# FrancisTheCat/raytracing_c

Hardware: AMD Instinct MI355X
Metric: Mray/s (higher is better)
Workload: dtype f32; 1 GPU; helmet.glb 1920x1080, 256 spp, 8 bounces (BASELINE.json configs[2]); partition=single GPU

## Files before the change

include/rt_hip.h:

```cpp
#ifndef RT_HIP_H
#define RT_HIP_H

#include "rt_raytracer.h"
#include "rt_materials.h"

#ifdef __cplusplus
extern "C" {
#endif

extern char const *rt_last_error(void);
extern void        rt_clear_error(void);

extern int rt_init(int device);

extern int rt_set_devices(i32 n_devices, i32 rehearse);
extern i32 rt_device_count(void);


extern void rt_set_seed(u32 seed);
extern u32  rt_get_seed(void);


typedef struct RT_Device_Scene RT_Device_Scene;

// ... 121 lines not shown


typedef struct {
  f32 alpha;
  i32 max_history;
  f32 normal_tolerance, plane_tolerance;
  i32 demodulate;
} RT_Temporal_Params;

typedef struct { f32 *color, *length, *coverage, *normal, *position; } RT_History_Planes;

extern i64 rt_temporal_history_bytes(i32 width, i32 height);
extern int rt_temporal_accumulate(i32 width, i32 height, RT_Temporal_Params const *params, Camera const *camera,
                                  Camera const *previous_camera, void const *d_color, void const *d_coverage, void const *d_albedo,
                                  void const *d_normal, void const *d_position, void const *d_history_in, void *d_history_out,
                                  void *d_out, void *d_length, void *d_image, void *stream);
extern int rt_temporal_accumulate_host(i32 width, i32 height, RT_Temporal_Params const *params, Camera const *camera,
                                       Camera const *previous_camera, f32 const *color, RT_Features const *planes,
                                       RT_History_Planes const *history_in, RT_History_Planes const *history_out, f32 *out,
                                       f32 *length, u8 *image);

typedef struct RT_History RT_History;
extern RT_History *rt_history_create(i32 width, i32 height);
extern int         rt_history_reset(RT_History *history);
extern void        rt_history_destroy(RT_History *history);

extern int rt_render_temporal(Scene const *scene, Image const *image, isize samples, isize max_bounces, RT_History *history,
                              RT_Temporal_Params const *temporal_params, RT_Guided_Params const *guided_params, f32 *linear_noisy,
                              f32 *linear_out, f32 *length);

extern int rt_get_counters(RT_Counters *out);
extern int rt_get_skipped_root_visits(u64 *out);
extern int rt_get_leafless_paths(u64 *out);

typedef struct {
  f32 stamp_ms, upload_ms, enqueue_ms, gpu_prep_ms, gpu_path_ms, gpu_resolve_ms, gpu_copy_ms, total_ms;
  f32 verify_ms;
  f32 gather_ms;
  i32 n_devices;
  i32 slowest_device;
} RT_Frame_Timing;
extern int rt_get_frame_timing(RT_Frame_Timing *out);

extern f32 rt_last_kernel_ms(void);

extern void rt_kernel_timing_reset(void);
extern f32  rt_kernel_timing_mean_ms(i32 *n_launches);

extern int rt_math_contract(void);


#ifdef __cplusplus
}
#endif

#endif
```

raytracing_c_amd/csrc/rt_dev.hip.h:

```cpp
#ifndef RT_DEV_HIP_H
#define RT_DEV_HIP_H

#include <hip/hip_runtime.h>
#include <stdint.h>

#include "rt_device.h"
#include "../../include/rt_math.h"

#define RT_BLOCK_WAVES 4
#define RT_BLOCK_THREADS (RT_BLOCK_WAVES * 64)

#define CNT_PATHS 0
#define CNT_RAYS 1
#define CNT_NODES 2
#define CNT_LEAVES 3
#define CNT_SHADES 4
#define CNT_BG 5
#define CNT_TEXTURED 6
#define CNT_SKIPPED_ROOT 7

struct Ray3 {
  rt_v3 o, d;
  float inv_x, inv_y, inv_z;
  bool  fast;
};

__device__ __forceinline__ rt_v3 slab_bias3(const Ray3 &r) {
#ifdef RT_MATH_NO_FMA
  return rt_v3_make(0.0f, 0.0f, 0.0f);
#else
  float px, py, pz;
  asm volatile("v_mul_f32 %0, %1, %2" : "=v"(px) : "v"(r.o.x), "v"(r.inv_x));
  asm volatile("v_mul_f32 %0, %1, %2" : "=v"(py) : "v"(r.o.y), "v"(r.inv_y));
  asm volatile("v_mul_f32 %0, %1, %2" : "=v"(pz) : "v"(r.o.z), "v"(r.inv_z));
  return rt_v3_make(-px, -py, -pz);
#endif
}

struct HitRec {
  float t;
  int   tri;
  float u, v;
};

struct LaneCounters {
  uint32_t rays, nodes, leaves, shades, bgs, textured, paths;
};

enum {
  LG_S_ITER = 0, LG_ENV_X, LG_ENV_L, LG_SHADE_X, LG_SHADE_L, LG_PSTORE_X, LG_PSTORE_L, LG_PLOAD_X, LG_PLOAD_L, LG_ACCUM_X, LG_ACCUM_L,
  LG_REGEN_X, LG_REGEN_L, LG_START_X, LG_START_L, LG_PRIM_X, LG_PRIM_L, LG_TILE_X, LG_JOIN_X, LG_FLUSH_X, LG_GRAB_X, LG_ROUND_X, LG_TRAV_CALLS,
  LG_NFULL_X, LG_NFULL_L, LG_NFULL_CAM, LG_NGLOB_X, LG_NGLOB_L, LG_NEXACT_X, LG_NEXACT_L, LG_CULLMASK_X, LG_PYRCHK_X, LG_NODE_WAIT_L,
  LG_NFEW0_X, LG_NFEW1_X, LG_NFEW2_X, LG_NFEW3_X, LG_NFEW4_X, LG_NFEW0_L, LG_NFEW1_L, LG_NFEW2_L, LG_NFEW3_L, LG_NFEW4_L,
  LG_LEAF_X, LG_LEAF_L, LG_LEAF_CAM, LG_POP_X, LG_POP_L, LG_POP_UP_L, LG_POP_RETEST_L, LG_POP_CAM, LG_POP_UP_X, LG_POP_RETEST_X, LG_POP_DONE_L,
  LG_CYC_S, LG_CYC_NODE, LG_CYC_LEAF, LG_CYC_POP, LG_CYC_WAVE, LG_CYC_TILE,
  LG_SKY_X, LG_SKY_L, LG_CYC_SKY,
  LG_CYC_COPY, LG_CYC_JOIN, LG_CYC_DRAIN, LG_DRAIN_X, LG_DRAIN_L, LG_CYC_FLUSH,
  LG_N
};
#define RT_LEDGER_ROW 128
#ifdef RT_LEDGER
__device__ __forceinline__ int lane_now();
__device__ __forceinline__ void lg_add(uint32_t *lg, int slot, uint32_t n) {
  if (lane_now() == 0 && n != 0u) __hip_atomic_fetch_add(lg + slot, n, __ATOMIC_RELAXED, __HIP_MEMORY_SCOPE_AGENT);
}
#define LG(slot, n) lg_add(lg, (slot), (uint32_t)(n))
#define LG_ARG , lg
#else
#define LG(slot, n) ((void)0)
#define LG_ARG
#endif
#ifdef RT_LEDGER_MARKS
#define LGM(name) asm volatile("; LEDGER_MARK " name)
#else
#define LGM(name) ((void)0)
#endif
#if defined(RT_LEDGER) && RT_LEDGER >= 2
#define LGT0() const unsigned long long lg_t0 = __builtin_amdgcn_s_memtime()
#define LGT1(slot) LG((slot), (uint32_t)((__builtin_amdgcn_s_memtime() - lg_t0) >> 4))
#define LGD0(n_live) do { if (!lg_drain_t0) { lg_drain_t0 = __builtin_amdgcn_s_memtime(); LG(LG_DRAIN_X, 1); LG(LG_DRAIN_L, (n_live)); } } while (0)
#define LGD1() do { if (lg_drain_t0) { LG(LG_CYC_DRAIN, (uint32_t)((__builtin_amdgcn_s_memtime() - lg_drain_t0) >> 4)); lg_drain_t0 = 0ull; } } while (0)
#else
#define LGT0() ((void)0)
#define LGT1(slot) ((void)0)
#define LGD0(n_live) ((void)0)
#define LGD1() ((void)0)
#endif

__device__ __forceinline__ float4 ld4(const float *base, int idx4) {
  return reinterpret_cast<const float4 *>(base)[idx4];
// ... 778 lines not shown

__device__ __forceinline__ uint32_t pyramid_cull_mask(const float4 *lds_nodes, const float *pyr, int node) {
  const int lane = lane_now();
  const float *nb = reinterpret_cast<const float *>(lds_nodes + lds_node_f4(node)) + (lane & 7);
  const float *pl = pyr + ((lane >> 3) & 3) * 4;
  const float ox = pyr[16], oy = pyr[17], oz = pyr[18];
  const float mnx = nb[0], mny = nb[8], mnz = nb[16], mxx = nb[24], mxy = nb[32], mxz = nb[40];
  const float nx = pl[0], ny = pl[1], nz = pl[2];
  const bool empty = mnx == 0.0f && mny == 0.0f && mnz == 0.0f && mxx == 0.0f && mxy == 0.0f && mxz == 0.0f;
  const float lox = nx * (mnx - ox), hix = nx * (mxx - ox), loy = ny * (mny - oy), hiy = ny * (mxy - oy);
  const float loz = nz * (mnz - oz), hiz = nz * (mxz - oz);
  const float nearest = fminf(lox, hix) + fminf(loy, hiy) + fminf(loz, hiz);
  const float extent = fmaxf(fabsf(lox), fabsf(hix)) + fmaxf(fabsf(loy), fabsf(hiy)) + fmaxf(fabsf(loz), fabsf(hiz));
  const float coarse = fabsf(nx) * (fabsf(ox) + fmaxf(fabsf(mnx), fabsf(mxx))) + fabsf(ny) * (fabsf(oy) + fmaxf(fabsf(mny), fabsf(mxy))) +
                       fabsf(nz) * (fabsf(oz) + fmaxf(fabsf(mnz), fabsf(mxz)));
  const bool outside = empty || nearest > 1e-3f * extent + 1e-6f * coarse;
  const uint32_t m = (uint32_t)__ballot(outside);
  return (m | (m >> 8) | (m >> 16) | (m >> 24)) & 0xFFu;
}

__device__ __forceinline__ float slab_entry_ordered(const Ray3 &r, const rt_v3 &bs, const char *nbase, int k, int nx, int ny, int nz, float t_max) {
  const char *b = nbase + k * 4;
  const float sx = rt_slab_t_fast(*reinterpret_cast<const float *>(b + nx), r.o.x, r.inv_x, bs.x);
  const float bx = rt_slab_t_fast(*reinterpret_cast<const float *>(b + (96 - nx)), r.o.x, r.inv_x, bs.x);
  const float sy = rt_slab_t_fast(*reinterpret_cast<const float *>(b + 32 + ny), r.o.y, r.inv_y, bs.y);
  const float by = rt_slab_t_fast(*reinterpret_cast<const float *>(b + 32 + (96 - ny)), r.o.y, r.inv_y, bs.y);
  const float sz = rt_slab_t_fast(*reinterpret_cast<const float *>(b + 64 + nz), r.o.z, r.inv_z, bs.z);
  const float bz = rt_slab_t_fast(*reinterpret_cast<const float *>(b + 64 + (96 - nz)), r.o.z, r.inv_z, bs.z);
  const float t_minv = fmax_hw(RT_EPS, fmax_hw(sx, fmax_hw(sy, sz)));
  const float t_maxv = fmin_hw(t_max, fmin_hw(bx, fmin_hw(by, bz)));
  return (t_minv < t_maxv) ? t_minv : RT_INF;
}

__device__ __forceinline__ uint32_t node_enter_few(const Ray3 &r, const float4 *lds_nodes, int node, uint32_t surv,
                                                   float hit_t) {
  const char *nbase = reinterpret_cast<const char *>(lds_nodes + lds_node_f4(node));
  const int nx = (as_i(r.inv_x) >> 31) & 96, ny = (as_i(r.inv_y) >> 31) & 96, nz = (as_i(r.inv_z) >> 31) & 96;
  const rt_v3 bs = slab_bias3(r);
  const int n = (int)__popc(surv);
  const int k0 = (int)__builtin_ctz(surv);
  const int e0 = as_i(slab_entry_ordered(r, bs, nbase, k0, nx, ny, nz, hit_t));
  const uint32_t f0 = 1u - (((uint32_t)e0 + 0x00800000u) >> 31);
  LGM("nfew_ret1");
  if (n == 1) return (uint32_t)k0 | (f0 << 24);
  surv &= surv - 1u;
  const int k1 = (int)__builtin_ctz(surv);
  const int e1 = as_i(slab_entry_ordered(r, bs, nbase, k1, nx, ny, nz, hit_t));
  const uint32_t f1 = 1u - (((uint32_t)e1 + 0x00800000u) >> 31);
  LGM("nfew_two");
  if (n == 2) {
    const bool swap = e1 < e0;
    const uint32_t first = swap ? (uint32_t)k1 : (uint32_t)k0, second = swap ? (uint32_t)k0 : (uint32_t)k1;
    return first | (second << 3) | ((f0 + f1) << 24);
  }
  LGM("nfew_ret2");
  surv &= surv - 1u;
  const int k2 = (int)__builtin_ctz(surv);
  const int e2 = as_i(slab_entry_ordered(r, bs, nbase, k2, nx, ny, nz, hit_t));
  const uint32_t f2 = 1u - (((uint32_t)e2 + 0x00800000u) >> 31);
  int e3 = 0x7F800000, k3 = 0;
  uint32_t f3 = 0;
  LGM("nfew_four_begin");
  if (n == 4) {
    surv &= surv - 1u;
    k3 = (int)__builtin_ctz(surv);
      e3 = as_i(slab_entry_ordered(r, bs, nbase, k3, nx, ny, nz, hit_t));
    f3 = 1u - (((uint32_t)e3 + 0x00800000u) >> 31);
  }
  LGM("nfew_four_end");
  const int e[4] = {e0, e1, e2, e3};
  const int kk[4] = {k0, k1, k2, k3};
  int rank[4] = {0, 1, 2, 3};
#pragma unroll
  for (int j = 0; j < 4; j++) {
#pragma unroll
    for (int k = j + 1; k < 4; k++) {
      int kb = (int)((uint32_t)(e[k] - e[j]) >> 31);
      rank[j] += kb;
      rank[k] -= kb;
    }
  }
  uint32_t w = 0;
#pragma unroll
  for (int j = 0; j < 4; j++) w |= (uint32_t)kk[j] << (3 * rank[j]);
  return w | ((f0 + f1 + f2 + f3) << 24);
}

__device__ __forceinline__ uint32_t pyramid_cull_tris(const float *leaves, const float *pyr, int g) {
  const int lane = lane_now();
  const float *tb = leaves + (size_t)g * 72 + (lane & 7);
  const float *pl = pyr + ((lane >> 3) & 3) * 4;
  const float ox = pyr[16], oy = pyr[17], oz = pyr[18];
  const float nx = pl[0], ny = pl[1], nz = pl[2];
  const float ax = tb[0], e1x = tb[8], e2x = tb[16], ay = tb[24], e1y = tb[32], e2y = tb[40], az = tb[48], e1z = tb[56], e2z = tb[64];
  bool outside = true;
#pragma unroll
  for (int v = 0; v < 3; v++) {
    const float vx = v == 0 ? ax : (v == 1 ? ax + e1x : ax + e2x);
    const float vy = v == 0 ? ay : (v == 1 ? ay + e1y : ay + e2y);
    const float vz = v == 0 ? az : (v == 1 ? az + e1z : az + e2z);
    const float px = nx * (vx - ox), py = ny * (vy - oy), pz = nz * (vz - oz);
    const float val = px + py + pz;
    const float extent = fabsf(px) + fabsf(py) + fabsf(pz);
    const float coarse = fabsf(nx) * (fabsf(ox) + fabsf(vx)) + fabsf(ny) * (fabsf(oy) + fabsf(vy)) + fabsf(nz) * (fabsf(oz) + fabsf(vz));
    outside = outside && (val > 1e-3f * extent + 1e-6f * coarse);
  }
  const uint32_t m = (uint32_t)__ballot(outside);
  return (m | (m >> 8) | (m >> 16) | (m >> 24)) & 0xFFu;
}

template <bool SHORT_DIV>
__device__ __forceinline__ void tri_test_uniform(const Ray3 &r, rt_v3 a, rt_v3 edge1, rt_v3 edge2, int k, float &best, float &bu, float &bv, int &bi) {
  rt_v3 rxe2 = rt_v3_cross(r.d, edge2);
  float det = rt_v3_dot(edge1, rxe2);
  float inv_det = SHORT_DIV ? rcp_leaf(det) : 1.0f / det;
  rt_v3 s = rt_v3_sub(r.o, a);
  rt_v3 sxe1 = rt_v3_cross(s, edge1);
  float u = inv_det * rt_v3_dot(s, rxe2);
  float v = inv_det * rt_v3_dot(r.d, sxe1);
// ... 21 lines not shown
  }
  if (best < hit.t) {
    hit.t = best;
    hit.tri = g * 8 + bi;
    hit.u = bu;
    hit.v = bv;
    return true;
  }
  return false;
}

typedef const RT_KParams __attribute__((address_space(4))) *RT_KArgs;
__device__ __forceinline__ RT_KArgs cold_args() {
  RT_KArgs p = (RT_KArgs)__builtin_amdgcn_kernarg_segment_ptr();
  asm volatile("" : "+s"(p));
  return p;
}

struct TravState {
  int      phase, level, node, child;
  uint32_t cur, dirty, live;
  HitRec   hit;
};

template <bool LDSN, bool SHORT_DIV, bool PYRAMID, bool ANY = false>
__device__ __forceinline__ void traversal_blocks(const RT_KParams &P, float4 *smem, const float4 *lds_nodes, uint32_t *perm,
                                                 const int lane, const int n_lds, const int pyr_nodes, const int pyr_off,
                                                 const int leaf_level, const int exit_lanes, const int n_trav0, const Ray3 &ray,
                                                 const bool is_cam, int &phase, int &level, int &node, int &child, uint32_t &cur,
                                                 uint32_t &dirty, uint32_t &live, HitRec &hit, uint32_t &w_nodes, uint32_t &w_leaves,
                                                 uint32_t *lg = nullptr) {
  static_assert(!(ANY && PYRAMID), "the pyramid-culled leaf block has no any-hit exit");
  LG(LG_TRAV_CALLS, 1);
  for (;;) {
    LGM("round_begin");
    const unsigned long long maskN = __ballot(phase == PH_NODE);
    const int nN = (int)__popcll(maskN);
    const int nL = (int)__popcll(__ballot(phase == PH_LEAF));
    if (nN + nL == 0 || n_trav0 - (nN + nL) >= exit_lanes) break;
    LG(LG_ROUND_X, 1);

    if (nL >= nN) {
      LGT0();
      LGM("leaf_begin");
      LG(LG_LEAF_X, 1); LG(LG_LEAF_L, nL);
#ifdef RT_LEDGER
      LG(LG_LEAF_CAM, __popcll(__ballot(phase == PH_LEAF && is_cam)));
#endif
      w_leaves += (uint32_t)nL;
      bool leaf_done = false;
      if (PYRAMID && pyr_nodes > 0) {
        const unsigned long long maskL = __ballot(phase == PH_LEAF);
        const unsigned long long camL = maskL & __ballot(is_cam);
        if (camL != 0ull) {
          const int c0 = __builtin_amdgcn_readlane(child, (int)__builtin_ctzll(camL));
          const int nG = (int)__popcll(camL & __ballot(child == c0));
          const int g0 = c0 - P.last_row_offset;
          if (nG * RT_PYR_DEN >= nL * RT_PYR_NUM && nG >= RT_PYR_MIN && (uint32_t)g0 < 0x800000u) {
            float *pyr = lds_at(smem, pyr_off);
            uint32_t *slot = reinterpret_cast<uint32_t *>(pyr) + 24 + (g0 & 7);
            const uint32_t key = 0x800000u | (uint32_t)g0;
            const uint32_t ce = (uint32_t)__builtin_amdgcn_readfirstlane((int)*slot);
            uint32_t cull;
            if ((ce >> 8) == key) {
              cull = ce & 0xFFu;
            } else {
              cull = pyramid_cull_tris(P.leaves, pyr, g0);
              if (lane_now() == 0) *slot = (key << 8) | cull;
            }
            if (__popc(0xFFu & ~cull) <= RT_LEAF_CULL_MAX) {
              w_leaves -= (uint32_t)(nL - nG);
              if (phase == PH_LEAF && is_cam && child == c0) {
                if (leaf_test_uniform<SHORT_DIV>(P, ray, g0, 0xFFu & ~cull, hit)) dirty = 0xFFFFFFFFu;
                phase = PH_POP;
              }
              leaf_done = true;
            }
          }
        }
// ... 18 lines not shown
        if (LDSN && all_fast && camN != 0ull) {
          const int c0 = __builtin_amdgcn_readlane(child, (int)__builtin_ctzll(camN));
          const int nG = (int)__popcll(camN & __ballot(child == c0));
          LG(LG_PYRCHK_X, 1);
          if (c0 < pyr_nodes && nG * RT_PYR_DEN >= nN * RT_PYR_NUM && nG >= RT_PYR_MIN) {
            float *pyr = lds_at(smem, pyr_off);
            uint32_t *slot = reinterpret_cast<uint32_t *>(pyr) + 32 + (c0 & 31);
            const uint32_t ce = (uint32_t)__builtin_amdgcn_readfirstlane((int)*slot);
            if ((ce >> 8) == (uint32_t)c0 + 1u) {
              surv = 0xFFu & ~ce;
            } else {
              LG(LG_CULLMASK_X, 1);
              LGM("cullmask_begin");
              const uint32_t cull = pyramid_cull_mask(lds_nodes, pyr, c0);
              if (lane_now() == 0) *slot = (((uint32_t)c0 + 1u) << 8) | cull;
              surv = 0xFFu & ~cull;
              LGM("cullmask_end");
            }
            if (__popc(surv) > 4) surv = 0xFFFFu;
            else {
              in_blk = phase == PH_NODE && is_cam && child == c0; w_nodes -= (uint32_t)(nN - nG);
#ifdef RT_LEDGER
              {
                const int ns = (int)__popc(surv);
                LG(LG_NFEW0_X, ns == 0); LG(LG_NFEW1_X, ns == 1); LG(LG_NFEW2_X, ns == 2); LG(LG_NFEW3_X, ns == 3); LG(LG_NFEW4_X, ns == 4);
                LG(LG_NFEW0_L, ns == 0 ? nG : 0); LG(LG_NFEW1_L, ns == 1 ? nG : 0); LG(LG_NFEW2_L, ns == 2 ? nG : 0);
                LG(LG_NFEW3_L, ns == 3 ? nG : 0); LG(LG_NFEW4_L, ns == 4 ? nG : 0); LG(LG_NODE_WAIT_L, nN - nG);
              }
#endif
            }
          }
        }
      }
      if (in_blk) {
        if (level >= 0) {
          perm[level * 64 + lane] = cur;
          live = (cur >> 24) ? (live | (1u << level)) : (live & ~(1u << level));
        }
        node = child;
        level += 1;
        if (PYRAMID && surv <= 0xFFu) {
          LGM("nfew_begin");
          cur = surv ? node_enter_few(ray, lds_nodes, node, surv, hit.t) : 0u;
          LGM("nfew_end");
        } else if (all_fast) {
          if (LDSN && __ballot(node >= n_lds) == 0) {
            LG(LG_NFULL_X, 1); LG(LG_NFULL_L, nN);
#ifdef RT_LEDGER
            LG(LG_NFULL_CAM, __popcll(maskN & __ballot(is_cam)));
#endif
            LGM("nfull_begin");
            cur = node_enter<true, NODE_LDS_ORDERED>(P, ray, node, hit.t, lds_nodes);
            LGM("nfull_end");
          } else {
            LG(LG_NGLOB_X, 1); LG(LG_NGLOB_L, nN);
            LGM("nglob_begin");
            cur = node_enter<true, NODE_GLOBAL>(P, ray, node, hit.t, lds_nodes);
            LGM("nglob_end");
          }
        } else if (ray.fast) {
          LGM("nexact_begin");
          LG(LG_NEXACT_X, 1); LG(LG_NEXACT_L, nN);
          cur = node_enter<true, NODE_GLOBAL>(P, ray, node, hit.t, lds_nodes);
        } else {
          cur = node_enter<false, NODE_GLOBAL>(P, ray, node, hit.t, lds_nodes);
        }
// ... 115 lines not shown
```

raytracing_c_amd/csrc/rt_device.h:

```cpp
#ifndef RT_DEVICE_H
#define RT_DEVICE_H

#include <stdint.h>

#define RT_NODE_F4   12
#define RT_LEAF_F4   18
#define RT_TRI_F4     7
#define RT_MAT_F4     9
#define RT_MAT_FLOATS 36
#define RT_MAX_DEPTH  8

#define RT_LDS_BYTES            (160 * 1024)
#define RT_LDS_NODE_BYTES       208
#define RT_LDS_TABLE_BYTES      64
#define RT_LDS_PERM_LEVEL_BYTES 256
#define RT_LDS_ACC_TILE_BYTES   1536

#define RT_MAT_DISNEY 0
#define RT_MAT_DEBUG  1

#define RT_TILE      8
#define RT_TILE_PIX  64

#define RT_PARK_RECORD_DWORDS (18 * 128)
#define RT_N_COUNTERS 137
#define RT_CNT_LEAFLESS 136



typedef struct {
  uint32_t offset;
  int32_t  width, height, stride;
} RT_DTexture;
#define RT_TEX_TILE_INDEX(x, y, tpr) ((((y) >> 2) * (tpr) + ((x) >> 2)) * 16 + (((y) & 3) << 2) + ((x) & 3))

typedef struct RT_KView {
  float    cam[3][4];
  float    focal_length;
  uint32_t seed;
  uint32_t pad[2];
} RT_KView;

typedef struct {
  const float    *nodes;
  const float    *leaves;
  const float    *tris;
  const float    *mats;
  const RT_DTexture *textures;
  const uint32_t *texels;
  int32_t depth;
  int32_t last_row_offset;
  int32_t bg_texture;
  int32_t n_nodes;
  float cam[3][4];
  float focal_length;
  float inv_width, inv_height, aspect;
  int32_t width, height, samples, max_bounces;
  int32_t sample_first, sample_end;
  uint32_t seed;
// ... 93 lines not shown
```

raytracing_c_amd/csrc/rt_kernels.hip:

```cpp

#include "rt_dev.hip.h"


#ifdef RT_LEDGER
#define RT_LEDGER_WAVES 8192
__device__ uint32_t g_ledger[RT_LEDGER_WAVES * RT_LEDGER_ROW];
__global__ void rt_ledger_reduce_kernel(unsigned long long *counters) {
  const int slot = threadIdx.x;
  if (slot >= LG_N || slot >= RT_LEDGER_ROW) return;
  unsigned long long sum = 0ull;
  for (int w = 0; w < RT_LEDGER_WAVES; w++) sum += g_ledger[w * RT_LEDGER_ROW + slot];
  counters[8 + slot] = sum;
}
#endif

typedef const RT_KView __attribute__((address_space(4))) *RT_KViewP;
template <bool VIEWS> struct CamSrc { typedef RT_KArgs type; };
template <> struct CamSrc<true> { typedef RT_KViewP type; };

template <int WAVES, bool LDSN, int MIN_WAVES_PER_SIMD, bool SHORT_DIV, bool VIEWS>
__global__ __launch_bounds__(WAVES * 64, MIN_WAVES_PER_SIMD) void rt_path_kernel_stream(RT_KParams P) {
  extern __shared__ float4 smem[];
  const int lane = threadIdx.x & 63;
  const int wave = threadIdx.x >> 6;
  const int n_lds = LDSN ? P.n_lds_nodes : 0;
  const float4 *lds_nodes = smem;
  const int perm_f4 = (P.depth > 0 ? P.depth : 1) * 16;
  float4 *wave_base = smem + n_lds * RT_LDS_NODE_F4 + wave * (perm_f4 + 96);
  uint32_t *perm = reinterpret_cast<uint32_t *>(wave_base);
  unsigned long long *acc = reinterpret_cast<unsigned long long *>(wave_base + perm_f4);
  const int acc_off = (n_lds * RT_LDS_NODE_F4 + __builtin_amdgcn_readfirstlane(wave) * (perm_f4 + 96) + perm_f4) * 16;
  const int pyr_off = (n_lds * RT_LDS_NODE_F4 + __builtin_amdgcn_readfirstlane(wave) * (perm_f4 + 96) + perm_f4 - 16) * 16;

#ifdef RT_LEDGER
  uint32_t *lg = g_ledger + (size_t)__builtin_amdgcn_readfirstlane((int)blockIdx.x * WAVES + wave) * RT_LEDGER_ROW;
  const unsigned long long lg_wave_t0 = __builtin_amdgcn_s_memtime();
#if RT_LEDGER >= 2
  unsigned long long lg_drain_t0 = 0ull;
#endif
#endif
  pow24_lds_init((int)threadIdx.x);
  if (LDSN) {
    LGT0();
    const float4 *g = reinterpret_cast<const float4 *>(P.nodes);
    for (int i = threadIdx.x; i < n_lds * 12; i += WAVES * 64) {
      int nd = i / 12, q = i - nd * 12;
      smem[nd * RT_LDS_NODE_F4 + q] = g[i];
    }
    __syncthreads();
    LGT1(LG_CYC_COPY);
  } else {
    __syncthreads();
  }

  acc[lane] = 0ull;
  acc[lane + 64] = 0ull;
  acc[lane + 128] = 0ull;

  uint32_t w_paths = 0, w_rays = 0, w_nodes = 0, w_leaves = 0, w_shades = 0, w_bgs = 0, w_tex = 0;
  const unsigned long long t_wave_start = cold_args()->wave_times ? __builtin_amdgcn_s_memrealtime() : 0ull;
  uint32_t n_tiles_done = 0;
  unsigned long long t_last_grab = 0ull;

  const int shift = P.chunk_shift;
  const int unit_paths = 2 << shift;
  const uint32_t n_chunks_tile = (uint32_t)P.n_chunks_tile;
  const int leaf_level = P.depth - 1;
  const int thresh = P.sched_thresh;
  const int drain_thresh = P.drain_thresh;
  const int pyr_nodes = LDSN ? P.pyr_nodes : 0;
  const int wave_id = (int)blockIdx.x * WAVES + wave;

  bool queue_open = true;
  int  steal_tries = 0;

  for (;;) {
    LGT0();
    LGM("tile_begin");
    int tile_idx = -1;
    if (queue_open) {
      RT_KArgs A = cold_args();
      uint32_t pos = 0;
      if (lane == 0) pos = atomicAdd(A->work_head, 1u);
      pos = (uint32_t)__builtin_amdgcn_readfirstlane((int)pos);
      const uint32_t *order = A->order;
      if (pos < (uint32_t)A->n_tiles) tile_idx = order ? (int)order[pos] : (int)pos;
      else queue_open = false;
    }
    if (tile_idx < 0) {
      if (steal_tries >= RT_STEAL_TRIES) break;
// ... 105 lines not shown
      if (lane < 40) reinterpret_cast<uint32_t *>(pyr)[24 + lane] = 0u;
      bool may_hit = false;
      if (lane < 8) {
        const float *nb = P.nodes + lane;
        rt_v3 lo = rt_v3_make(nb[0] - o.x, nb[8] - o.y, nb[16] - o.z);
        rt_v3 hi = rt_v3_make(nb[24] - o.x, nb[32] - o.y, nb[40] - o.z);
        const bool empty = nb[0] == 0.0f && nb[8] == 0.0f && nb[16] == 0.0f && nb[24] == 0.0f && nb[32] == 0.0f && nb[40] == 0.0f;
        bool outside = empty;
#pragma unroll
        for (int q = 0; q < 4; q++) {
          rt_v3 n = pn[q];
          float lox = n.x * lo.x, hix = n.x * hi.x, loy = n.y * lo.y, hiy = n.y * hi.y, loz = n.z * lo.z, hiz = n.z * hi.z;
          float nearest = fminf(lox, hix) + fminf(loy, hiy) + fminf(loz, hiz);
          float extent = fmaxf(fabsf(lox), fabsf(hix)) + fmaxf(fabsf(loy), fabsf(hiy)) + fmaxf(fabsf(loz), fabsf(hiz));
          float coarse = fabsf(n.x) * (fabsf(o.x) + fmaxf(fabsf(nb[0]), fabsf(nb[24]))) + fabsf(n.y) * (fabsf(o.y) + fmaxf(fabsf(nb[8]), fabsf(nb[32]))) +
                         fabsf(n.z) * (fabsf(o.z) + fmaxf(fabsf(nb[16]), fabsf(nb[40])));
          if (nearest > 1e-3f * extent + 1e-6f * coarse) outside = true;
        }
        may_hit = !outside;
      }
      tile_root_miss = __ballot(may_hit) == 0ull;
    }
#define RT_LEAFLESS_MAX 8
    int n_list = 0;
    int ll_levels = leaf_level, ll_nodes = pyr_nodes, ll_leaf0 = P.last_row_offset;
    asm volatile("" : "+s"(ll_levels), "+s"(ll_nodes), "+s"(ll_leaf0));
    if (ll_levels >= 1 && ll_nodes > 0 && !tile_root_miss) {
      const float *pyr = lds_at(smem, pyr_off);
      uint32_t *list = reinterpret_cast<uint32_t *>(lds_at(smem, pyr_off) - ll_levels * (RT_LDS_PERM_LEVEL_BYTES / 4));
      n_list = 1;
      for (int head = 0; head < n_list; head++) {
        const int nd = head ? __builtin_amdgcn_readfirstlane((int)list[RT_LEAFLESS_MAX + head]) : 0;
        const uint32_t surv = 0xFFu & ~pyramid_cull_mask(lds_nodes, pyr, nd);
        if (surv) {
          const int ns = (int)__popc(surv);
          if (8 * nd + 1 >= ll_leaf0 || 8 * nd + 8 >= ll_nodes || ns > 4 || n_list + ns > RT_LEAFLESS_MAX) { n_list = 0; break; }
          const int k = lane_now();
          if (k < 8 && ((surv >> k) & 1u)) {
            const int at = n_list + (int)__popc(surv & ((1u << k) - 1u));
            list[at] = (uint32_t)(nd * RT_LDS_NODE_BYTES + k * 4) | ((uint32_t)head << 20) | 0x80000000u;
            list[RT_LEAFLESS_MAX + at] = (uint32_t)(8 * nd + 1 + k);
          }
          n_list += ns;
        }
      }
    }
    const uint32_t rays_before = w_rays;
    LG(LG_TILE_X, 1);
    LGM("tile_end");
    LGT1(LG_CYC_TILE);

    int   phase = PH_NEED;
    int   pix = 0, bounce = 0;
    uint32_t rng = 0;
    Ray3  ray;
    ray_setup(ray, rt_v3_make(0, 0, 0), rt_v3_make(0, 0, 1));
    rt_v3 tint = rt_v3_make(1, 1, 1), emis = rt_v3_make(0, 0, 0);
    int   level = -1, node = 0, child = 0;
    uint32_t cur = 0, dirty = 0, live = 0;
    HitRec hit;
    hit.t = RT_INF; hit.tri = -1; hit.u = 0; hit.v = 0;

    bool tile_open = true;
    int  c_next = 0, c_end = 0, c_x0 = 0, c_y = 0, c_pix0 = 0, c_s0 = 0;
    uint32_t u_cur = 0, u_end = 0, grab = queue_open ? (uint32_t)cold_args()->grab_max : 1u;
    bool took_any = false;
// ... 294 lines not shown
          { const int n_pr = (int)__popcll(__ballot(got)); LG(LG_PRIM_X, n_pr != 0); LG(LG_PRIM_L, n_pr); LG(LG_REGEN_L, n_pr); }
#endif
          LGM("prim_begin");
          if (got) {
            typename CamSrc<VIEWS>::type S;
            if constexpr (VIEWS) S = vrec; else S = A;
            pix = gp;
            bounce = 0;
            rng = rt_path_seed(S->seed, (uint32_t)(gx + gy * width), (uint32_t)gs);
            PrimaryParams PP;
#pragma unroll
            for (int i = 0; i < 3; i++)
#pragma unroll
              for (int j = 0; j < 4; j++) PP.cam[i][j] = S->cam[i][j];
            PP.focal_length = S->focal_length; PP.inv_width = A->inv_width; PP.inv_height = A->inv_height; PP.aspect = A->aspect;
            primary_ray(PP, gx, gy, gs, org, dir);
            tint = rt_v3_make(1, 1, 1);
            emis = rt_v3_make(0, 0, 0);
            start = true;
            fresh = true;
          }
          LGM("prim_end");
        }
        bool skip_root = false;
#ifdef RT_LEDGER
        { const int n_st = (int)__popcll(__ballot(start)); LG(LG_START_X, n_st != 0); LG(LG_START_L, n_st); }
#endif
        LGM("start_begin");
        if (start) {
          ray_setup<SHORT_DIV>(ray, org, dir);
          hit.t = RT_INF; hit.tri = -1; hit.u = 0; hit.v = 0;
          dirty = 0;
          live = 0;
          cur = 0;
          level = -1;
          node = 0;
          child = (leaf_level >= 0) ? 0 : P.last_row_offset;
          phase = (leaf_level >= 0) ? PH_NODE : PH_LEAF;
          skip_root = fresh && tile_root_miss && ray.fast;
          if (skip_root) phase = PH_MISS;
        }
        LGM("start_end");
        w_rays += (uint32_t)__popcll(__ballot(start));
        {
          const uint32_t n_skip = (uint32_t)__popcll(__ballot(skip_root));
          w_nodes += n_skip;
          if (n_skip != 0u && lane == 0) atomicAdd(cold_args()->counters + CNT_SKIPPED_ROOT, (unsigned long long)n_skip);
        }
        LGM("s_end");
        LGT1(LG_CYC_S);
      }

      const int n_trav0 = (int)__popcll(__ballot(phase == PH_NODE || phase == PH_LEAF));
      if (n_trav0 == 0) {
        if (__any(phase == PH_MISS)) continue;
        if (n_parked > 0 || __any(phase == PH_HIT)) continue;
        if (!tile_open) break;
        continue;
      }

      traversal_blocks<LDSN, SHORT_DIV, true>(P, smem, lds_nodes, perm, lane, n_lds, pyr_nodes, pyr_off, leaf_level,
                                              tile_open ? thresh : drain_thresh, n_trav0, ray, bounce == 0, phase, level, node,
                                              child, cur, dirty, live, hit, w_nodes, w_leaves LG_ARG);
    }

    LGD1();
    LGM("flush_begin");
    if (took_any) {
      LGT0();
      LG(LG_FLUSH_X, 1);
      int x = tile_x0 + (lane & 7), y = tile_y0 + (lane >> 3);
      unsigned long long r = acc[lane * 3 + 0], g = acc[lane * 3 + 1], b = acc[lane * 3 + 2];
      acc[lane * 3 + 0] = 0ull;
      acc[lane * 3 + 1] = 0ull;
      acc[lane * 3 + 2] = 0ull;
      RT_KArgs A = cold_args();
      const int width = A->width;
      if (x < width && y < A->height && (r | g | b) != 0ull) {
        unsigned long long *base = A->accum;
        if constexpr (VIEWS) base += (size_t)(vrec - (RT_KViewP)A->views) * (size_t)A->pixels_per_view * 3;
        unsigned long long *dst = base + ((size_t)y * width + x) * 3;
        atomicAdd(dst + 0, r);
        atomicAdd(dst + 1, g);
        atomicAdd(dst + 2, b);
      }
      uint32_t *tile_cost = A->tile_cost;
      if (tile_cost && lane == 0) atomicAdd(&tile_cost[tile_idx], w_rays - rays_before);
      steal_tries = 0;
      n_tiles_done += 1;
      LGT1(LG_CYC_FLUSH);
    }
  }
  RT_KArgs A = cold_args();
  unsigned long long *wave_times = A->wave_times, *counters = A->counters;
  if (wave_times && lane == 0 && wave_id < 65536) {
    wave_times[wave_id * 3 + 0] = t_wave_start;
    wave_times[wave_id * 3 + 1] = __builtin_amdgcn_s_memrealtime();
    wave_times[wave_id * 3 + 2] = ((t_last_grab - t_wave_start) << 16) | (n_tiles_done & 0xFFFFu);
  }

  if (lane == 0) {
    atomicAdd(counters + CNT_PATHS, (unsigned long long)w_paths);
    atomicAdd(counters + CNT_RAYS, (unsigned long long)w_rays);
    atomicAdd(counters + CNT_NODES, (unsigned long long)w_nodes);
    atomicAdd(counters + CNT_LEAVES, (unsigned long long)w_leaves);
    atomicAdd(counters + CNT_SHADES, (unsigned long long)w_shades);
    atomicAdd(counters + CNT_BG, (unsigned long long)w_bgs);
    atomicAdd(counters + CNT_TEXTURED, (unsigned long long)w_tex);
#ifdef RT_LEDGER
    LG(LG_CYC_WAVE, (uint32_t)((__builtin_amdgcn_s_memtime() - lg_wave_t0) >> 4));
#endif
  }
}

__global__ void rt_resolve_kernel(int width, int height, int samples, int chunks_x, const int32_t *local_chunks,
                                  int n_local_chunks, const unsigned long long *accum,
                                  uint8_t *tiles, uint8_t *image, float *linear) {
  int idx = blockIdx.x * blockDim.x + threadIdx.x;
  if (idx >= n_local_chunks * 1024) return;
  int lchunk = idx >> 10, p = idx & 1023;
// ... 469 lines not shown
```

raytracing_c_amd/csrc/rt_launch.cpp:

```cpp

#include "rt_host.h"

int check_params(RT_Render_Params const *p) {
  if (!p) return rt_fail("render params are NULL");
  if (p->width <= 0 || p->height <= 0) return rt_fail("image size %dx%d is invalid", p->width, p->height);
  if ((int64_t)p->width * p->height > (int64_t)1 << 28) return rt_fail("image %dx%d is too large", p->width, p->height);
  if (p->samples <= 0) return rt_fail("samples must be positive (got %d)", p->samples);
  if (p->max_bounces < 0) return rt_fail("max_bounces must be >= 0 (got %d)", p->max_bounces);
  if (p->world <= 0 || p->rank < 0 || p->rank >= p->world) return rt_fail("rank %d / world %d is invalid", p->rank, p->world);
  if (p->sample_first < 0 || p->sample_count < 0 || p->sample_first + p->sample_count > p->samples)
    return rt_fail("sample range [%d, +%d) outside [0, %d)", p->sample_first, p->sample_count, p->samples);
  return 0;
}

int check_image_size(const char *who, i32 width, i32 height) {
  if (width <= 0 || height <= 0) return rt_fail("%s: image size %dx%d is invalid", who, width, height);
  if ((int64_t)width * height > RT_MAX_PIXELS) return rt_fail("%s: image %dx%d is too large (more than 2^28 pixels)", who, width, height);
  return 0;
}

int check_views(i32 n_views, RT_View const *views, i32 width, i32 height, const char *who) {
  if (n_views <= 0) return rt_fail("%s: n_views must be positive (got %d)", who, n_views);
  if (!views) return rt_fail("%s: views is NULL", who);
  if (width <= 0 || height <= 0) return rt_fail("%s: image size %dx%d is invalid", who, width, height);
// ... 361 lines not shown
  } else {
    std::vector<uint8_t> tmp(pixels * 3);
    HIP_TRY(hipMemcpy(tmp.data(), d_image, pixels * 3, hipMemcpyDeviceToHost));
    for (isize y = 0; y < image->height; y++)
      for (isize x = 0; x < image->width; x++)
        for (int c = 0; c < 3; c++)
          image->pixels.data[image->components * (x + y * image->stride) + c] = tmp[((size_t)y * width + x) * 3 + c];
  }
  return 0;
}

extern "C" int rt_get_skipped_root_visits(u64 *out) {
  if (!out) return rt_fail("rt_get_skipped_root_visits: NULL");
  Device &D = dev0();
  std::lock_guard<std::mutex> lock(D.mutex);
  if (ensure_device(D) != 0) return -1;
  unsigned long long c[RT_N_COUNTERS];
  if (read_counters(D, c) != 0) return -1;
  *out = c[7];
  return 0;
}

extern "C" int rt_get_leafless_paths(u64 *out) {
  if (!out) return rt_fail("rt_get_leafless_paths: NULL");
  Device &D = dev0();
  std::lock_guard<std::mutex> lock(D.mutex);
  if (ensure_device(D) != 0) return -1;
  unsigned long long c[RT_N_COUNTERS];
  if (read_counters(D, c) != 0) return -1;
  *out = c[RT_CNT_LEAFLESS];
  return 0;
}

int read_counters(Device &D, unsigned long long c[RT_N_COUNTERS]) {
  HIP_TRY(hipDeviceSynchronize());
  if (!D.last_counters) { memset(c, 0, RT_N_COUNTERS * sizeof(unsigned long long)); return 0; }
  HIP_TRY(hipMemcpy(c, D.last_counters, RT_N_COUNTERS * sizeof(unsigned long long), hipMemcpyDeviceToHost));
  return 0;
}

extern "C" int rt_get_counters(RT_Counters *out) {
  if (!out) return rt_fail("rt_get_counters: NULL");
  {
    std::lock_guard<std::mutex> lk(g_multi_mutex);
    if (g_multi_counters_valid) { *out = g_multi_counters; return 0; }
  }
  Device &D = dev0();
  std::lock_guard<std::mutex> lock(D.mutex);
  if (ensure_device(D) != 0) return -1;
  unsigned long long c[RT_N_COUNTERS];
  if (read_counters(D, c) != 0) return -1;
  out->paths = c[0];
  out->rays = c[1];
  out->node_visits = c[2];
  out->leaf_visits = c[3];
  out->shades = c[4];
  out->backgrounds = c[5];
  out->textured = c[6];
  return 0;
}

static float timed_slot_ms(Workspace &W, size_t slot) {
  if (hipEventSynchronize(W.ev1[slot]) != hipSuccess) return -1.0f;
  return event_ms(W.ev0[slot], W.ev1[slot]);
}

// ... 30 lines not shown
```

raytracing_c_amd/ctypes_abi.py:

```python
import ctypes as C

import numpy as np

isize = C.c_ssize_t
f32 = C.c_float


class Vec2(C.Structure):
    _fields_ = [("x", f32), ("y", f32)]


class Vec3(C.Structure):
    _fields_ = [("x", f32), ("y", f32), ("z", f32)]


class Matrix_4x4(C.Structure):
    _fields_ = [("rows", (f32 * 4) * 4)]


class Byte_Slice(C.Structure):
    _fields_ = [("data", C.c_void_p), ("len", isize)]


class Image(C.Structure):
# ... 155 lines not shown
assert RAY_HIT_DTYPE.itemsize == C.sizeof(RT_Ray_Hit) == 16
assert DEVICE_HIT_DTYPE.itemsize == C.sizeof(RT_Device_Hit) == 88
assert HIT_DTYPE.itemsize == C.sizeof(Hit) == 88
RT_QUERY_MAX_RAYS = 1 << 30
RT_QUERY_SLICE = 1 << 20

assert C.sizeof(BVH_Node) == 192
assert C.sizeof(Triangle) == 112
assert C.sizeof(Triangle_AOS) == 112
assert C.sizeof(Hit) == 88
assert C.sizeof(PBR_Shader_Data) == 80

TRIANGLE_DTYPE = np.dtype([("positions", "<f4", (3, 3)), ("normals", "<f4", (3, 3)), ("tex_coords", "<f4", (3, 2)),
                           ("shader_data", "<u8"), ("shader_proc", "<u8")])
assert TRIANGLE_DTYPE.itemsize == 112

EXPORTED_SYMBOLS = [
    "render_thread_proc", "rendering_context_is_finished", "rendering_context_finish", "lightmap_bake", "render",
    "denoise_image",
    "scene_init", "scene_init_sah", "scene_init_gpu", "rt_scene_alloc", "rt_scene_free", "scene_load_bytes", "scene_save_bytes", "scene_file_size",
    "rt_scene_slot_map", "scene_refit", "scene_refit_gpu",
    "disney_shader_proc", "debug_shader_proc", "sample_background",
    "rt_last_error", "rt_clear_error", "rt_init", "rt_set_seed", "rt_get_seed",
    "rt_set_devices", "rt_device_count", "rt_math_contract",
    "rt_scene_verify", "rt_scene_touch", "rt_scene_set_static", "rt_get_frame_timing",
    "rt_scene_upload", "rt_scene_release", "rt_scene_invalidate", "rt_scene_device_bytes", "rt_set_camera",
    "rt_chunk_count", "rt_chunk_owner", "rt_local_chunk_count", "rt_max_local_chunk_count", "rt_local_chunk_list", "rt_render_accumulate", "rt_resolve", "rt_untile",
    "rt_denoise", "rt_render_frame", "rt_frame_begin", "rt_frame_end", "rt_render_views", "rt_render_accumulate_views",
    "rt_query_closest", "rt_query_occluded", "rt_scene_hits", "rt_scene_closest", "rt_scene_occluded", "rt_get_query_counters",
    "rt_render_accumulate_features", "rt_resolve_features", "rt_render_features",
    "rt_guided_work_bytes", "rt_guided_denoise", "rt_guided_denoise_host", "rt_render_denoised",
    "rt_temporal_history_bytes", "rt_temporal_accumulate", "rt_temporal_accumulate_host", "rt_history_create", "rt_history_reset",
    "rt_history_destroy", "rt_render_temporal",
    "rt_get_counters", "rt_get_skipped_root_visits", "rt_get_leafless_paths", "rt_last_kernel_ms", "rt_kernel_timing_reset", "rt_kernel_timing_mean_ms",
]

DIAG_ONLY_SYMBOLS = [
    "rt_diag_set_tokens", "rt_diag_multi_fault", "rt_set_pipeline", "rt_get_pipeline", "rt_set_wavefront_capacity", "rt_get_wave_times", "rt_get_ledger",
    "rt_diag_device_bytes_live", "rt_diag_release_staging",
    "rt_test_math", "rt_test_rcp_sweep", "rt_test_srgb_sweep", "rt_test_quantize_sweep", "rt_test_trace", "rt_test_trace_stream",
    "rt_test_tile_order", "rt_test_texture", "rt_test_shade", "rt_test_brdf", "rt_test_background", "rt_test_primary_ray",
]
```

raytracing_c_amd/native.py:

```python
import ctypes as C
import os

from . import ctypes_abi as abi

_HERE = os.path.dirname(os.path.abspath(__file__))
LIB_PATH = os.environ.get("RT_LIB_PATH") or os.path.join(_HERE, "librt_hip.so")
DIAG_PATH = os.path.join(_HERE, "librt_hip_diag.so")


class NativeLibraryMissing(RuntimeError):
    pass


def _preload_hip_runtime():
    import importlib.util
    import sys
    if os.environ.get("RT_HIP_RUNTIME", "torch") != "torch":
        return
    if "torch" in sys.modules:
        return
    try:
        spec = importlib.util.find_spec("torch")
    except (ImportError, ValueError):
        spec = None
# ... 94 lines not shown
        d.rt_query_occluded.argtypes = [vp, C.c_int64, vp, vp, vp, vp]
        d.rt_scene_hits.argtypes = [P(abi.Scene), C.c_int64, vp, vp, vp]
        d.rt_scene_closest.argtypes = [P(abi.Scene), C.c_int64, vp, vp, vp]
        d.rt_scene_occluded.argtypes = [P(abi.Scene), C.c_int64, vp, vp, vp]
        d.rt_get_query_counters.argtypes = [P(abi.RT_Query_Counters)]
    if hasattr(d, "rt_render_features"):
        d.rt_render_accumulate_features.argtypes = [vp, P(abi.RT_Render_Params), vp, vp]
        d.rt_resolve_features.argtypes = [P(abi.RT_Render_Params), vp, vp, vp, vp, vp, vp]
        d.rt_render_features.argtypes = [P(abi.Scene), C.c_int32, C.c_int32, abi.isize, abi.isize, P(abi.RT_Features), vp]
    if hasattr(d, "rt_guided_denoise"):
        d.rt_guided_work_bytes.argtypes = [C.c_int32, C.c_int32]
        d.rt_guided_work_bytes.restype = C.c_int64
        d.rt_guided_denoise.argtypes = [C.c_int32, C.c_int32, P(abi.RT_Guided_Params)] + [vp] * 9
        d.rt_guided_denoise_host.argtypes = [C.c_int32, C.c_int32, P(abi.RT_Guided_Params), vp, P(abi.RT_Features), vp, vp]
        d.rt_render_denoised.argtypes = [P(abi.Scene), P(abi.Image), abi.isize, abi.isize, P(abi.RT_Guided_Params), vp, vp]
    if hasattr(d, "rt_temporal_accumulate"):
        d.rt_temporal_history_bytes.argtypes = [C.c_int32, C.c_int32]
        d.rt_temporal_history_bytes.restype = C.c_int64
        d.rt_temporal_accumulate.argtypes = [C.c_int32, C.c_int32, P(abi.RT_Temporal_Params), P(abi.Camera), P(abi.Camera)] + [vp] * 11
        d.rt_temporal_accumulate_host.argtypes = [C.c_int32, C.c_int32, P(abi.RT_Temporal_Params), P(abi.Camera), P(abi.Camera), vp,
                                                  P(abi.RT_Features), P(abi.RT_History_Planes), P(abi.RT_History_Planes), vp, vp, vp]
        d.rt_history_create.argtypes = [C.c_int32, C.c_int32]
        d.rt_history_create.restype = vp
        d.rt_history_reset.argtypes = [vp]
        d.rt_history_destroy.argtypes = [vp]
        d.rt_history_destroy.restype = None
        d.rt_render_temporal.argtypes = [P(abi.Scene), P(abi.Image), abi.isize, abi.isize, vp, P(abi.RT_Temporal_Params),
                                         P(abi.RT_Guided_Params), vp, vp, vp]
    d.rt_get_counters.argtypes = [P(abi.RT_Counters)]
    if hasattr(d, "rt_get_skipped_root_visits"):
        d.rt_get_skipped_root_visits.argtypes = [P(C.c_uint64)]
    if hasattr(d, "rt_get_leafless_paths"):
        d.rt_get_leafless_paths.argtypes = [P(C.c_uint64)]
    d.rt_math_contract.restype = C.c_int
    d.rt_last_kernel_ms.restype = C.c_float
    d.rt_kernel_timing_reset.restype = None
    d.rt_kernel_timing_mean_ms.argtypes = [P(C.c_int32)]
    d.rt_kernel_timing_mean_ms.restype = C.c_float
    d.rt_set_devices.argtypes = [C.c_int32, C.c_int32]
    d.rt_device_count.restype = C.c_int32
    d.rt_scene_verify.argtypes = [P(abi.Scene)]
    d.rt_scene_touch.argtypes = [P(abi.Scene), vp, C.c_size_t]
    d.rt_scene_set_static.argtypes = [P(abi.Scene), C.c_int32]
    d.rt_scene_set_static.restype = None
    d.rt_get_frame_timing.argtypes = [P(abi.RT_Frame_Timing)]
    d.render_thread_proc.argtypes = [P(abi.Rendering_Context)]
    d.render_thread_proc.restype = None
    d.rendering_context_is_finished.argtypes = [P(abi.Rendering_Context)]
    d.rendering_context_is_finished.restype = C.c_bool
    d.rendering_context_finish.argtypes = [P(abi.Rendering_Context)]
    d.rendering_context_finish.restype = None
    d.render.argtypes = [P(abi.Scene), P(abi.Image), abi.isize, abi.isize]
    d.lightmap_bake.argtypes = [P(abi.Image), P(abi.Scene), abi.isize]
    d.lightmap_bake.restype = None
    d.denoise_image.argtypes = [P(abi.Image), P(abi.Image), abi.isize]
    d.denoise_image.restype = None
    d.rt_denoise.argtypes = [C.c_int32, C.c_int32, vp, vp, vp]


def _declare_diag(d):
    vp = C.c_void_p
    d.rt_test_math.argtypes = [C.c_int32, C.c_int32, vp, vp, vp]
    d.rt_test_rcp_sweep.argtypes = [vp]
    d.rt_test_srgb_sweep.argtypes = [vp]
    d.rt_test_quantize_sweep.argtypes = [vp]
    d.rt_test_trace.argtypes = [vp, C.c_int32, vp, vp, vp, vp]
# ... 33 lines not shown
```

Baseline: 22260 Mray/s.

## Fuse BVH root visit into path loop with precomputed populated-child mask

At kernel start, computes which of the root's 8 children are populated and, when four or fewer are, stores that mask in LDS. Rays starting at the root then take a fused wave-level step that enters the root through node_enter_few with that mask, skipping the generic traversal block for the root. Primary-bounce waves can also reuse a cached pyramid cull mask from the leafless-list precompute. This adds LDS bookkeeping, a shared atomic counter for fused root visits, and new ledger diagnostics, and it relies on the populated-child detection being correct.

Measured after the change: 22500 Mray/s (median of 6 runs). 1.01x the previous value.

```diff
diff --git a/include/rt_hip.h b/include/rt_hip.h
--- a/include/rt_hip.h
+++ b/include/rt_hip.h
@@ -177,6 +177,7 @@
 extern int rt_get_counters(RT_Counters *out);
 extern int rt_get_skipped_root_visits(u64 *out);
 extern int rt_get_leafless_paths(u64 *out);
+extern int rt_get_fused_root_visits(u64 *out);
 
 typedef struct {
   f32 stamp_ms, upload_ms, enqueue_ms, gpu_prep_ms, gpu_path_ms, gpu_resolve_ms, gpu_copy_ms, total_ms;
diff --git a/raytracing_c_amd/csrc/rt_dev.hip.h b/raytracing_c_amd/csrc/rt_dev.hip.h
--- a/raytracing_c_amd/csrc/rt_dev.hip.h
+++ b/raytracing_c_amd/csrc/rt_dev.hip.h
@@ -56,6 +56,7 @@
   LG_CYC_S, LG_CYC_NODE, LG_CYC_LEAF, LG_CYC_POP, LG_CYC_WAVE, LG_CYC_TILE,
   LG_SKY_X, LG_SKY_L, LG_CYC_SKY,
   LG_CYC_COPY, LG_CYC_JOIN, LG_CYC_DRAIN, LG_DRAIN_X, LG_DRAIN_L, LG_CYC_FLUSH,
+  LG_ROOT_FULL_X, LG_ROOT_FULL_L, LG_ROOT_CULL_X, LG_ROOT_CULL_L, LG_ROOT_LEFT_X, LG_ROOT_LEFT_L, LG_ROOTF_X, LG_ROOTF_L,
   LG_N
 };
 #define RT_LEDGER_ROW 128
@@ -900,6 +901,8 @@
   return (t_minv < t_maxv) ? t_minv : RT_INF;
 }
 
+#define LGM_FEW(name) do { if (AT_ROOT) LGM("rfew_" name); else LGM("nfew_" name); } while (0)
+template <bool AT_ROOT = false>
 __device__ __forceinline__ uint32_t node_enter_few(const Ray3 &r, const float4 *lds_nodes, int node, uint32_t surv,
                                                    float hit_t) {
   const char *nbase = reinterpret_cast<const char *>(lds_nodes + lds_node_f4(node));
@@ -909,33 +912,33 @@
   const int k0 = (int)__builtin_ctz(surv);
   const int e0 = as_i(slab_entry_ordered(r, bs, nbase, k0, nx, ny, nz, hit_t));
   const uint32_t f0 = 1u - (((uint32_t)e0 + 0x00800000u) >> 31);
-  LGM("nfew_ret1");
+  LGM_FEW("ret1");
   if (n == 1) return (uint32_t)k0 | (f0 << 24);
   surv &= surv - 1u;
   const int k1 = (int)__builtin_ctz(surv);
   const int e1 = as_i(slab_entry_ordered(r, bs, nbase, k1, nx, ny, nz, hit_t));
   const uint32_t f1 = 1u - (((uint32_t)e1 + 0x00800000u) >> 31);
-  LGM("nfew_two");
+  LGM_FEW("two");
   if (n == 2) {
     const bool swap = e1 < e0;
     const uint32_t first = swap ? (uint32_t)k1 : (uint32_t)k0, second = swap ? (uint32_t)k0 : (uint32_t)k1;
     return first | (second << 3) | ((f0 + f1) << 24);
   }
-  LGM("nfew_ret2");
+  LGM_FEW("ret2");
   surv &= surv - 1u;
   const int k2 = (int)__builtin_ctz(surv);
   const int e2 = as_i(slab_entry_ordered(r, bs, nbase, k2, nx, ny, nz, hit_t));
   const uint32_t f2 = 1u - (((uint32_t)e2 + 0x00800000u) >> 31);
   int e3 = 0x7F800000, k3 = 0;
   uint32_t f3 = 0;
-  LGM("nfew_four_begin");
+  LGM_FEW("four_begin");
   if (n == 4) {
     surv &= surv - 1u;
     k3 = (int)__builtin_ctz(surv);
       e3 = as_i(slab_entry_ordered(r, bs, nbase, k3, nx, ny, nz, hit_t));
     f3 = 1u - (((uint32_t)e3 + 0x00800000u) >> 31);
   }
-  LGM("nfew_four_end");
+  LGM_FEW("four_end");
   const int e[4] = {e0, e1, e2, e3};
   const int kk[4] = {k0, k1, k2, k3};
   int rank[4] = {0, 1, 2, 3};
@@ -953,6 +956,7 @@
   for (int j = 0; j < 4; j++) w |= (uint32_t)kk[j] << (3 * rank[j]);
   return w | ((f0 + f1 + f2 + f3) << 24);
 }
+#undef LGM_FEW
 
 __device__ __forceinline__ uint32_t pyramid_cull_tris(const float *leaves, const float *pyr, int g) {
   const int lane = lane_now();
@@ -1040,6 +1044,9 @@
                                                  uint32_t *lg = nullptr) {
   static_assert(!(ANY && PYRAMID), "the pyramid-culled leaf block has no any-hit exit");
   LG(LG_TRAV_CALLS, 1);
+#ifdef RT_LEDGER
+  bool lg_after_root_cull = false;
+#endif
   for (;;) {
     LGM("round_begin");
     const unsigned long long maskN = __ballot(phase == PH_NODE);
@@ -1053,6 +1060,7 @@
       LGM("leaf_begin");
       LG(LG_LEAF_X, 1); LG(LG_LEAF_L, nL);
 #ifdef RT_LEDGER
+      lg_after_root_cull = false;
       LG(LG_LEAF_CAM, __popcll(__ballot(phase == PH_LEAF && is_cam)));
 #endif
       w_leaves += (uint32_t)nL;
@@ -1137,6 +1145,18 @@
           }
         }
       }
+#ifdef RT_LEDGER
+      {
+        const unsigned long long mb = __ballot(in_blk);
+        const int nb = (int)__popcll(mb);
+        const bool root_blk = mb != 0ull && (mb & __ballot(child != 0)) == 0ull;
+        const bool culled = PYRAMID && surv <= 0xFFu;
+        LG(LG_ROOT_CULL_X, root_blk && culled); LG(LG_ROOT_CULL_L, root_blk && culled ? nb : 0);
+        LG(LG_ROOT_FULL_X, root_blk && !culled); LG(LG_ROOT_FULL_L, root_blk && !culled ? nb : 0);
+        LG(LG_ROOT_LEFT_X, root_blk && !culled && lg_after_root_cull); LG(LG_ROOT_LEFT_L, root_blk && !culled && lg_after_root_cull ? nb : 0);
+        lg_after_root_cull = root_blk && culled;
+      }
+#endif
       if (in_blk) {
         if (level >= 0) {
           perm[level * 64 + lane] = cur;
diff --git a/raytracing_c_amd/csrc/rt_device.h b/raytracing_c_amd/csrc/rt_device.h
--- a/raytracing_c_amd/csrc/rt_device.h
+++ b/raytracing_c_amd/csrc/rt_device.h
@@ -23,8 +23,9 @@
 #define RT_TILE_PIX  64
 
 #define RT_PARK_RECORD_DWORDS (18 * 128)
-#define RT_N_COUNTERS 137
+#define RT_N_COUNTERS 138
 #define RT_CNT_LEAFLESS 136
+#define RT_CNT_FUSED_ROOT 137
 
 
 
diff --git a/raytracing_c_amd/csrc/rt_kernels.hip b/raytracing_c_amd/csrc/rt_kernels.hip
--- a/raytracing_c_amd/csrc/rt_kernels.hip
+++ b/raytracing_c_amd/csrc/rt_kernels.hip
@@ -56,6 +56,21 @@
   acc[lane] = 0ull;
   acc[lane + 64] = 0ull;
   acc[lane + 128] = 0ull;
+
+  if (LDSN) {
+    uint32_t *pw = reinterpret_cast<uint32_t *>(lds_at(smem, pyr_off));
+    bool populated = false;
+    if (lane_now() < 8 && cold_args()->n_lds_nodes > 0 && cold_args()->depth > 0) {
+      const float *nb = lds_at(smem, 0) + lane_now();
+      populated = !(nb[0] == 0.0f && nb[8] == 0.0f && nb[16] == 0.0f && nb[24] == 0.0f && nb[32] == 0.0f && nb[40] == 0.0f);
+    }
+    const uint32_t pm = (uint32_t)__ballot(populated) & 0xFFu;
+#ifdef RT_ROOT_AT_NODE_BLOCKS
+    if (lane_now() == 0) { pw[19] = 0u; pw[20] = 0u; }
+#else
+    if (lane_now() == 0) { pw[19] = __popc(pm) <= 4 ? pm : 0u; pw[20] = 0u; }
+#endif
+  }
 
   uint32_t w_paths = 0, w_rays = 0, w_nodes = 0, w_leaves = 0, w_shades = 0, w_bgs = 0, w_tex = 0;
   const unsigned long long t_wave_start = cold_args()->wave_times ? __builtin_amdgcn_s_memrealtime() : 0ull;
@@ -227,6 +242,7 @@
       for (int head = 0; head < n_list; head++) {
         const int nd = head ? __builtin_amdgcn_readfirstlane((int)list[RT_LEAFLESS_MAX + head]) : 0;
         const uint32_t surv = 0xFFu & ~pyramid_cull_mask(lds_nodes, pyr, nd);
+        if (lane_now() == 0) reinterpret_cast<uint32_t *>(lds_at(smem, pyr_off))[32 + (nd & 31)] = ((uint32_t)(nd + 1) << 8) | (0xFFu & ~surv);
         if (surv) {
           const int ns = (int)__popc(surv);
           if (8 * nd + 1 >= ll_leaf0 || 8 * nd + 8 >= ll_nodes || ns > 4 || n_list + ns > RT_LEAFLESS_MAX) { n_list = 0; break; }
@@ -587,7 +603,7 @@
           hit.t = RT_INF; hit.tri = -1; hit.u = 0; hit.v = 0;
           dirty = 0;
           live = 0;
-          cur = 0;
+          cur = (LDSN && ray.fast && reinterpret_cast<const uint32_t *>(lds_at(smem, pyr_off))[19] != 0u) ? 1u : 0u;
           level = -1;
           node = 0;
           child = (leaf_level >= 0) ? 0 : P.last_row_offset;
@@ -612,6 +628,40 @@
         if (n_parked > 0 || __any(phase == PH_HIT)) continue;
         if (!tile_open) break;
         continue;
+      }
+
+      if (LDSN) {
+        const bool at_root = phase == PH_NODE && level < 0 && cur != 0u;
+        const int n_root = (int)__popcll(__ballot(at_root));
+        if (n_root != 0) {
+          LGM("root_begin");
+          LG(LG_ROOTF_X, 1); LG(LG_ROOTF_L, n_root);
+          uint32_t *pw = reinterpret_cast<uint32_t *>(lds_at(smem, pyr_off));
+          const uint32_t w_pop = pw[19], w_cull = pw[32];
+          uint32_t rsurv = (uint32_t)__builtin_amdgcn_readfirstlane((int)w_pop);
+          w_nodes += (uint32_t)n_root;
+          if (lane_now() == 0) {
+            const uint32_t at = (uint32_t)(uintptr_t)(__attribute__((address_space(3))) uint32_t *)(pw + 20);
+            asm volatile("ds_add_u32 %0, %1" : : "v"(at), "v"((uint32_t)n_root) : "memory");
+          }
+          if (__ballot(at_root && bounce != 0) == 0ull) {
+            const uint32_t ce = (uint32_t)__builtin_amdgcn_readfirstlane((int)w_cull);
+            if ((ce >> 8) == 1u) rsurv &= ~ce;
+          }
+          if (at_root) {
+            level = 0;
+            cur = rsurv ? node_enter_few<true>(ray, lds_nodes, 0, rsurv, RT_INF) : 0u;
+            if (cur >> 24) {
+              child = 1 + (int)(cur & 7u);
+              cur = ((cur >> 3) & 0x1FFFFFu) | (((cur >> 24) - 1u) << 24);
+              phase = (leaf_level == 0) ? PH_LEAF : PH_NODE;
+            } else {
+              level = -1;
+              phase = PH_MISS;
+            }
+          }
+          LGM("root_end");
+        }
       }
 
       traversal_blocks<LDSN, SHORT_DIV, true>(P, smem, lds_nodes, perm, lane, n_lds, pyr_nodes, pyr_off, leaf_level,
@@ -641,6 +691,12 @@
       }
       uint32_t *tile_cost = A->tile_cost;
       if (tile_cost && lane == 0) atomicAdd(&tile_cost[tile_idx], w_rays - rays_before);
+      if (LDSN && lane == 0) {
+        uint32_t *pw = reinterpret_cast<uint32_t *>(lds_at(smem, pyr_off));
+        const uint32_t n_fused = pw[20];
+        pw[20] = 0u;
+        if (n_fused != 0u) atomicAdd(A->counters + RT_CNT_FUSED_ROOT, (unsigned long long)n_fused);
+      }
       steal_tries = 0;
       n_tiles_done += 1;
       LGT1(LG_CYC_FLUSH);
diff --git a/raytracing_c_amd/csrc/rt_launch.cpp b/raytracing_c_amd/csrc/rt_launch.cpp
--- a/raytracing_c_amd/csrc/rt_launch.cpp
+++ b/raytracing_c_amd/csrc/rt_launch.cpp
@@ -417,6 +417,17 @@
   return 0;
 }
 
+extern "C" int rt_get_fused_root_visits(u64 *out) {
+  if (!out) return rt_fail("rt_get_fused_root_visits: NULL");
+  Device &D = dev0();
+  std::lock_guard<std::mutex> lock(D.mutex);
+  if (ensure_device(D) != 0) return -1;
+  unsigned long long c[RT_N_COUNTERS];
+  if (read_counters(D, c) != 0) return -1;
+  *out = c[RT_CNT_FUSED_ROOT];
+  return 0;
+}
+
 int read_counters(Device &D, unsigned long long c[RT_N_COUNTERS]) {
   HIP_TRY(hipDeviceSynchronize());
   if (!D.last_counters) { memset(c, 0, RT_N_COUNTERS * sizeof(unsigned long long)); return 0; }
diff --git a/raytracing_c_amd/ctypes_abi.py b/raytracing_c_amd/ctypes_abi.py
--- a/raytracing_c_amd/ctypes_abi.py
+++ b/raytracing_c_amd/ctypes_abi.py
@@ -211,7 +211,7 @@
     "rt_guided_work_bytes", "rt_guided_denoise", "rt_guided_denoise_host", "rt_render_denoised",
     "rt_temporal_history_bytes", "rt_temporal_accumulate", "rt_temporal_accumulate_host", "rt_history_create", "rt_history_reset",
     "rt_history_destroy", "rt_render_temporal",
-    "rt_get_counters", "rt_get_skipped_root_visits", "rt_get_leafless_paths", "rt_last_kernel_ms", "rt_kernel_timing_reset", "rt_kernel_timing_mean_ms",
+    "rt_get_counters", "rt_get_skipped_root_visits", "rt_get_leafless_paths", "rt_get_fused_root_visits", "rt_last_kernel_ms", "rt_kernel_timing_reset", "rt_kernel_timing_mean_ms",
 ]
 
 DIAG_ONLY_SYMBOLS = [
diff --git a/raytracing_c_amd/native.py b/raytracing_c_amd/native.py
--- a/raytracing_c_amd/native.py
+++ b/raytracing_c_amd/native.py
@@ -150,6 +150,8 @@
         d.rt_get_skipped_root_visits.argtypes = [P(C.c_uint64)]
     if hasattr(d, "rt_get_leafless_paths"):
         d.rt_get_leafless_paths.argtypes = [P(C.c_uint64)]
+    if hasattr(d, "rt_get_fused_root_visits"):
+        d.rt_get_fused_root_visits.argtypes = [P(C.c_uint64)]
     d.rt_math_contract.restype = C.c_int
     d.rt_last_kernel_ms.restype = C.c_float
     d.rt_kernel_timing_reset.restype = None
```
